# baldhat/yolov10-3D

Hardware: AMD Instinct MI355X
Metric: train_images_per_sec (higher is better)
Workload: dtype bf16

## Files before the change

include/y3d.h:

```cpp
#ifndef Y3D_H
#define Y3D_H
#include <stdint.h>

#ifdef __cplusplus
extern "C" {
#endif

enum { Y3D_F32 = 0, Y3D_BF16 = 1 };
enum { Y3D_OK = 0, Y3D_ERR_INVALID = -1, Y3D_ERR_HIP = -2 };

const char* y3d_last_error(void);
int y3d_abi_version(void);
int y3d_device_info(char* name, int name_len, int* compute_units, int* lds_bytes, int* clock_khz);

int y3d_pack_weight_fwd(int dtype, const float* w_oihw, void* out, int Cout, int Cin_g, int Cin_g_pad, int kh, int kw, void* stream);
int y3d_pack_weight_dgrad(int dtype, const float* w_oihw, void* out, int Cout, int Cin_g, int groups, int kh, int kw, void* stream);
int y3d_mt_pack_weights(int dtype, const int64_t* desc, const int* chunk_tensor, const int* chunk_off, int nchunks, int chunk, void* stream);
int y3d_mt_fp8w_quantize(const int64_t* desc, const int* row_begin, int ntensors, int nrows, void* stream);
int y3d_fp8w_dequantize(const uint8_t* codes, const float* scale, float* w, int rows, int K, void* stream);
int y3d_fp8_quantize_act(const void* x, int64_t xsw, int64_t M, int C, uint8_t* q, uint8_t* s, void* stream);
int y3d_fp8_pack_weight_fwd(const uint8_t* codes, const float* scale, int rows, int Cg, uint8_t* wq, uint8_t* ws, void* stream);
int y3d_conv3x3_fp8_ok(int B, int H, int W, int Cin, int Cout, int groups);
int y3d_conv3x3_fp8_stat_rows(int B, int H, int W);
int y3d_fp8_scale_pitch(int C);
// ... 15 lines not shown
  Y3D_ROUTE_SMALL = 2,
  Y3D_ROUTE_SMALL_S2 = 3,
  Y3D_ROUTE_S2_DGRAD = 4,
  Y3D_ROUTE_TILE8 = 5,
  Y3D_ROUTE_TILE16 = 6,
  Y3D_ROUTE_WIDE3_8 = 7,
  Y3D_ROUTE_WIDE3_16 = 8,
  Y3D_ROUTE_FLAT = 9,
  Y3D_ROUTE_WGRAD_SMALL = 10,
  Y3D_ROUTE_WGRAD_TILE = 11,
  Y3D_ROUTE_WGRAD_STREAM1X1 = 12
};
int y3d_conv2d_route(int dtype, int op, int epi, int B, int H, int W, int Cin, int Cout, int groups, int kh, int kw, int stride, int pad);
int y3d_conv2d_fwd(int dtype, const void* x, int64_t xsb, int64_t xsh, int64_t xsw, int B, int H, int W, int Cin,
                   const void* w_packed, const float* bias, void* y, int64_t ysw, int Ho, int Wo, int Cout, int groups,
                   int kh, int kw, int stride, int pad, float* stat_partials, void* stream);
int y3d_conv2d_fwd_affine(int dtype, const void* x, int64_t xsb, int64_t xsh, int64_t xsw, int B, int H, int W, int Cin,
                          const void* w_packed, const float* scale, const float* shift, int act, void* y, int64_t ysw, int Ho, int Wo,
                          int Cout, int groups, int kh, int kw, int stride, int pad, void* stream);
int y3d_conv2d_fwd_affine_res_ok(int dtype, int B, int H, int W, int Cin, int Cout, int groups, int kh, int kw, int stride, int pad);
int y3d_conv2d_fwd_affine_res(int dtype, const void* x, int64_t xsb, int64_t xsh, int64_t xsw, int B, int H, int W, int Cin,
                              const void* w_packed, const float* scale, const float* shift, int act, const void* res, int64_t rsw, void* y,
                              int64_t ysw, int Ho, int Wo, int Cout, int groups, int kh, int kw, int stride, int pad, void* stream);
int y3d_conv2d_bwd_data(int dtype, const void* dy, int64_t dsb, int64_t dsh, int64_t dsw, int B, int Ho, int Wo, int Cout,
                        const void* w_packed_dgrad, void* dx, int64_t xsw, int H, int W, int Cin, int groups, int kh, int kw,
                        int stride, int pad, void* stream);
int y3d_conv2d_wgrad_splits(int dtype, int B, int Ho, int Wo, int Cout, int Cin_g, int groups, int kh, int kw);
int y3d_conv2d_wgrad_plan(int dtype, int B, int H, int W, int Cin, int Cout, int groups, int kh, int kw, int stride, int pad);
int y3d_set_tile_kernels(int enable);
int y3d_set_stream1x1(int enable);
int y3d_get_stream1x1(void);
int y3d_get_tile_kernels(void);
int y3d_set_bn_wide_slabs(int enable);
int y3d_conv2d_bwd_weight(int dtype, const void* x, int64_t xsb, int64_t xsh, int64_t xsw, int B, int H, int W, int Cin,
                          int Cin_real, const void* dy, int64_t dsw, int Ho, int Wo, int Cout, int groups, int kh, int kw,
                          int stride, int pad, float* slab, int nsplit, float* grad_oihw, int accumulate, void* stream);
int y3d_wgrad_fold(const float* slab, int nsplit, int Cout, int taps, int Cin_g, int Cin_g_real, float* grad_oihw, int accumulate,
                   void* stream);

int y3d_dw_blocks(int64_t M);
int y3d_dw_wgrad_blocks(int64_t M);
int y3d_dw_pack_weight(const float* w_oihw, float* out_taps_c, int C, int kh, int kw, void* stream);
int y3d_dwconv2d_fwd(int dtype, const void* x, int64_t xsb, int64_t xsh, int64_t xsw, int B, int H, int W, int C,
                     const float* w_packed, void* y, int64_t ysw, int Ho, int Wo, int kh, int kw, int stride, int pad,
                     float* stat_partials, void* stream);
int y3d_dwconv2d_fwd_affine(int dtype, const void* x, int64_t xsb, int64_t xsh, int64_t xsw, int B, int H, int W, int C,
                            const float* w_packed, const float* scale, const float* shift, int act, int res_mode, const void* res, int64_t rsw,
                            void* z, int64_t zsw, int Ho, int Wo, int kh, int kw, int stride, int pad, void* stream);
int y3d_dwconv2d_bwd_data(int dtype, const void* dy, int64_t dsb, int64_t dsh, int64_t dsw, int B, int Ho, int Wo, int C,
                          const float* w_packed, void* dx, int64_t xsw, int H, int W, int kh, int kw, int stride, int pad,
                          void* stream);
int y3d_dwconv2d_bwd_weight(int dtype, const void* x, int64_t xsb, int64_t xsh, int64_t xsw, int B, int H, int W, int C,
                            const void* dy, int64_t dsw, int Ho, int Wo, int kh, int kw, int stride, int pad, float* slab,
                            float* grad_oihw, int accumulate, void* stream);
int y3d_dw_wgrad_fold(const float* slab, int nblk, int C, int taps, float* grad_oihw, int accumulate, void* stream);

int y3d_bn_finalize(const float* partials, int nblk, int C, int64_t count, const float* gamma, const float* beta, float eps,
                    float momentum, float* running_mean, float* running_var, float* mean, float* invstd, float* scale,
                    float* shift, void* stream);
int y3d_bn_eval_scale(int C, const float* gamma, const float* beta, const float* running_mean, const float* running_var,
                      float eps, float* scale, float* shift, void* stream);
int y3d_bn_act_fwd(int dtype, const void* y, int64_t ysw, const float* scale, const float* shift, int act, int res_mode,
                   const void* res, int64_t rsw, void* z, int64_t zsw, int64_t P, int C, void* stream);
int y3d_bn_act_fwd_q(const void* y, int64_t ysw, const float* scale, const float* shift, int act, void* z, int64_t zsw, uint8_t* q, uint8_t* s,
                     int64_t P, int C, void* stream);
int y3d_bn_bwd_blocks(int64_t P, int C);
// ... 220 lines not shown
```

yolov10-3d_amd/_lib.py:

```python
from __future__ import annotations

import ctypes
import os
import re

_HERE = os.path.dirname(os.path.abspath(__file__))
LIB_PATH = os.path.join(_HERE, "liby3d_hip.so")
HEADER = os.path.join(os.path.dirname(_HERE), "include", "y3d.h")

F32, BF16 = 0, 1

_CT = {"int": ctypes.c_int, "int64_t": ctypes.c_int64, "float": ctypes.c_float, "double": ctypes.c_double}


class Y3DError(RuntimeError):
    pass


def parse_header(path: str = HEADER):
    src = open(path).read()
    src = re.sub(r"/\*.*?\*/", " ", src, flags=re.S)
    protos = {}
    for m in re.finditer(r"(const\s+char\s*\*|int)\s+(y3d_\w+)\s*\(([^;{]*?)\)\s*;", src, flags=re.S):
        ret, name, args = m.group(1), m.group(2), m.group(3).strip()
        argtypes = []
        if args and args != "void":
            for a in args.split(","):
                a = a.strip()
                if "*" in a:
                    argtypes.append(ctypes.c_void_p)
                else:
                    toks = a.split()
                    t = toks[1] if toks[0] == "const" else toks[0]
                    argtypes.append(_CT[t])
        protos[name] = (ctypes.c_char_p if "char" in ret else ctypes.c_int, argtypes)
    return protos


_PLAIN_INT = {"abi_version", "conv_kpad", "conv_stat_blocks", "conv2d_stat_rows", "conv2d_route", "conv2d_wgrad_splits", "conv2d_wgrad_plan", "set_tile_kernels", "set_stream1x1", "set_bn_wide_slabs", "get_stream1x1", "get_tile_kernels", "dw_blocks", "dw_wgrad_blocks", "bn_bwd_blocks", "proj_blocks", "proj_group_blocks", "proj_group_bn_bwd_blocks", "proj_group_bwd_weight_bn_mfma_blocks", "tal3d_scratch_floats", "tal2d_scratch_floats", "v10_postprocess_scratch_floats", "conv2d_fwd_affine_res_ok", "stem_conv_train_rows", "conv3x3_fp8_ok", "conv3x3_fp8_dgrad_ok", "conv3x3_fp8_stat_rows", "fp8_scale_pitch", "kitti_eval_max_boxes", "det_metrics_max_gts", "det_metrics_max_dets"}


class _Lib:
    def __init__(self):
        if not os.path.exists(LIB_PATH):
            raise Y3DError(
                f"{LIB_PATH} not found: build it with `python yolov10-3d_amd/csrc/build.py` "
                "(or __graft_entry__.build()). There is no CPU / PyTorch fallback for the HIP path.")
        self._dll = ctypes.CDLL(LIB_PATH)
        self.protos = parse_header()
        for name, (ret, argtypes) in self.protos.items():
            fn = getattr(self._dll, name)
            fn.restype = ret
            fn.argtypes = argtypes

    def last_error(self) -> str:
        return (self._dll.y3d_last_error() or b"").decode()

    def __getattr__(self, name):
        if name.startswith("_"):
            raise AttributeError(name)
        fn = getattr(self._dll, "y3d_" + name)
        ret = self.protos["y3d_" + name][0]
        if ret is not ctypes.c_int or name in _PLAIN_INT:
            setattr(self, name, fn)
            return fn

        def call(*a):
            rc = fn(*a)
            if rc != 0:
                raise Y3DError(f"y3d_{name} failed ({rc}): {self.last_error()}")
            return rc

# ... 13 lines not shown
```

yolov10-3d_amd/csrc/conv3x3_wgrad_tile.hip:

```cpp
#include "common.h"
#include <cstdlib>

namespace {

__device__ uint4 y3d_wg_zero_page[4];

struct WG3P {
  const void* x;
  const void* dy;
  float* slab;
  long xsb, xsh, xsw, dsw;
  int B, H, W;
  int Cg, Cn, G;
  int ntx, nty;
  int ntiles, tiles_per_split, nslab;
};

typedef __attribute__((ext_vector_type(8))) short s16x8_t;

template <int OFF>
__device__ __forceinline__ s16x4_t ds_tr16(unsigned a) {
  s16x4_t v;
#ifdef Y3D_WGP_NOLDS
  asm volatile("" : "=v"(v) : "v"(a));
  return v;
#endif
  asm volatile("ds_read_b64_tr_b16 %0, %1 offset:%2" : "=v"(v) : "v"(a), "n"(OFF));
  return v;
}
template <int N>
__device__ __forceinline__ void lds_wait(s16x4_t& a, s16x4_t& b, s16x4_t& c, s16x4_t& d) {
  asm volatile("s_waitcnt lgkmcnt(%4)" : "+v"(a), "+v"(b), "+v"(c), "+v"(d) : "n"(N));
}

template <int N>
__device__ __forceinline__ void lds_wait8(s16x4_t& a, s16x4_t& b, s16x4_t& c, s16x4_t& d, s16x4_t& e, s16x4_t& f, s16x4_t& g, s16x4_t& h) {
  asm volatile("s_waitcnt lgkmcnt(%8)" : "+v"(a), "+v"(b), "+v"(c), "+v"(d), "+v"(e), "+v"(f), "+v"(g), "+v"(h) : "n"(N));
}

template <int TH>
__global__ __launch_bounds__(512) void conv3x3_wgrad_tile_kernel(WG3P p) {
  typedef bf16_t T;
  constexpr int NT = 512;
  constexpr int NPX = TH * 16;
  constexpr int HWD = 18;
  constexpr int NPIXH = (TH + 2) * HWD;
  constexpr int DR = NPX * 16 / NT;
  constexpr int HCH = NPIXH * 8;
  constexpr int HR = (HCH + NT - 1) / NT;
  constexpr int DBYTES = NPX * 256, HBYTES = HR * NT * 16, SBYTES = DBYTES + HBYTES;
  extern __shared__ __attribute__((aligned(16))) char smem[];

  const int tid = threadIdx.x, lane = tid & 63, wave = tid >> 6;
  const int wi = wave >> 1, wj = wave & 1;
  const int g = blockIdx.z, split = blockIdx.y;
  const int slab_i = blockIdx.x % p.nslab, cot = blockIdx.x / p.nslab;
  const int c0 = cot * 128, ci0 = slab_i * 64;
  const T* __restrict__ X = (const T*)p.x;
  const T* __restrict__ D = (const T*)p.dy;
  const T* zero = (const T*)y3d_wg_zero_page;

  int d_row[DR], d_px[DR], d_c[DR];
#pragma unroll
  for (int rd = 0; rd < DR; ++rd) {
    int chunk = rd * NT + tid;
    int pp = chunk >> 4, s = chunk & 15;
    d_row[rd] = pp >> 4;
    d_px[rd] = pp & 15;
    d_c[rd] = (s ^ ((pp & 7) << 1)) * 8;
  }
  int h_y[HR], h_x[HR], h_c[HR];
#pragma unroll
  for (int rd = 0; rd < HR; ++rd) {
    int chunk = rd * NT + tid;
    int P = chunk >> 3, s = chunk & 7;
    h_y[rd] = chunk < HCH ? P / HWD : -100000;
    h_x[rd] = P - (P / HWD) * HWD;
    h_c[rd] = (s ^ (((h_x[rd] >> 1) & 3) << 1)) * 8;
  }
  auto issue = [&](int tile, int buf) {
    int tx = tile % p.ntx;
    int t2 = tile / p.ntx;
    int ty = t2 % p.nty;
    int b = t2 / p.nty;
    const int x0 = tx * 16, y0 = ty * TH;
    char* db = smem + buf * SBYTES;
    char* hb = db + DBYTES;
#pragma unroll
    for (int rd = 0; rd < DR; ++rd) {
// ... 105 lines not shown
          for (int mt = 0; mt < 2; ++mt)
#pragma unroll
            for (int nt = 0; nt < 2; ++nt)
#ifndef Y3D_WGP_NOMFMA
              acc[r * 3 + q][mt][nt] = __builtin_amdgcn_mfma_f32_16x16x32_bf16(fa[mt], fb[nt], acc[r * 3 + q][mt][nt], 0, 0, 0);
#else
              asm volatile("" ::"v"(fa[mt]), "v"(fb[nt]));
#endif
        }
      }
    }
    asm volatile("s_waitcnt vmcnt(0)" ::: "memory");
    __syncthreads();
  }

  const int Ktot = 9 * p.Cg;
  float* slab = p.slab + ((long)split * p.G * p.Cn + (long)g * p.Cn) * Ktot;
#pragma unroll
  for (int tap = 0; tap < 9; ++tap)
#pragma unroll
    for (int mt = 0; mt < 2; ++mt)
#pragma unroll
      for (int nt = 0; nt < 2; ++nt) {
        int ci = ci0 + wj * 32 + nt * 16 + (lane & 15);
#pragma unroll
        for (int rg = 0; rg < 4; ++rg) {
          int co = c0 + wi * 32 + mt * 16 + (lane >> 4) * 4 + rg;
          if (co < p.Cn && ci < p.Cg) slab[(long)co * Ktot + tap * p.Cg + ci] = acc[tap][mt][nt][rg];
        }
      }
}

template <int TH>
int launch_wg(const WG3P& p, int nsplit, hipStream_t st) {
  constexpr int NPX = TH * 16;
  constexpr int HCH = (TH + 2) * 18 * 8;
  constexpr int HR = (HCH + 511) / 512;
  size_t sm = 2 * ((size_t)NPX * 256 + (size_t)HR * 512 * 16);
  static bool attr_set = false;
  if (!attr_set) {
    (void)hipFuncSetAttribute((const void*)conv3x3_wgrad_tile_kernel<TH>, hipFuncAttributeMaxDynamicSharedMemorySize, (int)sm);
    attr_set = true;
  }
  dim3 grid(p.nslab * cdiv(p.Cn, 128), nsplit, p.G);
  hipLaunchKernelGGL((conv3x3_wgrad_tile_kernel<TH>), grid, dim3(512), sm, st, p);
  Y3D_LAUNCH_CHECK();
  return Y3D_OK;
}

}

int y3d_wgrad_tile_height(int dtype, int H, int W, int Cg, int Cn, int kh, int kw, int stride, int pad) {
  if (dtype != Y3D_BF16 || kh != 3 || kw != 3 || stride != 1 || pad != 1) return 0;
  if (Cg % 16 != 0 || Cg < 64 || Cn % 8 != 0 || W < 8) return 0;
  if (H % 8 == 0) return 8;
  if (H % 4 == 0) return 4;
  return 0;
}

int y3d_wgrad_tile_splits(int th, int B, int H, int W, int Cg, int Cn, int G) {
  long ntiles = (long)B * (H / th) * cdiv(W, 16);
  long blocks = (long)cdiv(Cg, 64) * cdiv(Cn, 128) * G;
  const int target8 = 256;
  const long tgt = th == 8 ? target8 : 2 * target8;
  long want = tgt / blocks;
  if (want > ntiles) want = ntiles;
  long slab_bytes = (long)G * Cn * 9 * Cg * 4;
  long cap = (64L << 20) / slab_bytes;
  if (cap < 16) cap = 16;
  if (cap > 256) cap = 256;
  if (want > cap) want = cap;
  if (want < 1) want = 1;
  return (int)want;
}

int y3d_conv3x3_wgrad_tile_launch(int th, const void* x, long xsb, long xsh, long xsw, const void* dy, long dsw, int B, int H, int W, int Cg,
                                  int Cn, int G, float* slab, int nsplit, void* stream) {
// ... 13 lines not shown
```

yolov10-3d_amd/csrc/conv_gemm.hip:

```cpp
#include "common.h"
#include "conv_frag.h"
#include <cstdlib>

namespace {

struct ConvP {
  const void* x;
  const void* w;
  const float* bias;
  const float* scale;
  const float* shift;
  int act;
  void* y;
  float* part;
  long xsb, xsh, xsw;
  long ysw;
  int B, Hg, Wg;
  int Hq, Wq;
  int Cg, Cn, G;
  int kh, kw, stride, pad;
  int Ktot, Kpad;
  int M;
  int ntx, nty;
};
// ... 244 lines not shown
    for (int a = 0; a < TC; ++a)
#pragma unroll
      for (int j = 0; j < 4; ++j) {
        float s = wave_xor_sum16(ssum[a][j]);
        float q = wave_xor_sum16(ssq[a][j]);
        if (lp == 0) {
          int cl = wc * (BC / WC) + a * 16 + lc + j;
          red[(wp * BC + cl) * 2 + 0] = s;
          red[(wp * BC + cl) * 2 + 1] = q;
        }
      }
    __syncthreads();
    if (tid < BC && c0 + tid < p.Cn) {
      float s = 0.f, q = 0.f;
#pragma unroll
      for (int w = 0; w < WP; ++w) { s += red[(w * BC + tid) * 2]; q += red[(w * BC + tid) * 2 + 1]; }
      float* dst = p.part + ((long)tile_x * (p.G * p.Cn) + g * p.Cn + c0 + tid) * 2;
      dst[0] = s;
      dst[1] = q;
    }
  }
}

struct WgradP {
  const void* x;
  const void* dy;
  float* slab;
  long xsb, xsh, xsw;
  long dsw;
  int B, H, W, Ho, Wo;
  int Cg, Cn, G;
  int kh, kw, stride, pad;
  int Ktot, M, nsplit, chunk_px;
};

template <typename T, int W> struct TFrag;
template <int W> struct TFrag<bf16_t, W> {
  typedef bf16x8_t type;
  static constexpr int KSUB_PX = 32;
  static constexpr int PITCH = W * 2 + 32;
  __device__ static __forceinline__ type load(const char* tile, int i0, int k0, int lane) {
    int grp = lane >> 4, li = lane & 15;
    int q = li >> 2, pp = li & 3;
    const char* a0 = tile + (k0 + 4 * grp + q) * PITCH + (i0 + 4 * pp) * 2;
    s16x4_t lo = __builtin_amdgcn_ds_read_tr16_b64_v4i16((s16x4_t __attribute__((address_space(3)))*)(a0));
    s16x4_t hi = __builtin_amdgcn_ds_read_tr16_b64_v4i16((s16x4_t __attribute__((address_space(3)))*)(a0 + 16 * PITCH));
    typedef __attribute__((ext_vector_type(8))) short s16x8_t;
    s16x8_t v = __builtin_shufflevector(lo, hi, 0, 1, 2, 3, 4, 5, 6, 7);
    return __builtin_bit_cast(bf16x8_t, v);
  }
  __device__ static __forceinline__ f32x4_t mma(type a, type b, f32x4_t c) {
    return __builtin_amdgcn_mfma_f32_16x16x32_bf16(a, b, c, 0, 0, 0);
  }
};
template <int W> struct TFrag<float, W> {
  typedef float type;
  static constexpr int KSUB_PX = 4;
  static constexpr int PITCH = W * 4 + 64;
  __device__ static __forceinline__ type load(const char* tile, int i0, int k0, int lane) {
    return *(const float*)(tile + (k0 + (lane >> 4)) * PITCH + (i0 + (lane & 15)) * 4);
  }
  __device__ static __forceinline__ f32x4_t mma(type a, type b, f32x4_t c) {
    return __builtin_amdgcn_mfma_f32_16x16x4f32(a, b, c, 0, 0, 0);
  }
};

template <typename T, int WD, int WX>
__global__ __launch_bounds__(256) void conv_wgrad_kernel(WgradP p) {
  constexpr int CE = TT<T>::CE;
  constexpr int BPK = TT<T>::BKE;
  constexpr int PD = TFrag<T, WD>::PITCH, PX = TFrag<T, WX>::PITCH;
  constexpr int CPD = WD * sizeof(T) / 16, CPX = WX * sizeof(T) / 16;
  constexpr int ND = BPK * CPD / 256 > 0 ? BPK * CPD / 256 : 1;
  constexpr int NX = BPK * CPX / 256 > 0 ? BPK * CPX / 256 : 1;
  constexpr int TA = WD / 32, TB = WX / 32;
  extern __shared__ __attribute__((aligned(16))) char smem[];
  char* sD = smem;
  char* sX = smem + 2 * BPK * PD;

  const int tid = threadIdx.x, lane = tid & 63, wave = tid >> 6;
  const int wi = wave >> 1, wj = wave & 1;
  const int g = blockIdx.z % p.G;
  const int split = blockIdx.z / p.G;
  const int j0 = blockIdx.x * WX;
  const int i0 = blockIdx.y * WD;
  const T* __restrict__ X = (const T*)p.x;
  const T* __restrict__ D = (const T*)p.dy;

  const int mbeg = split * p.chunk_px;
  const int mend = min(p.M, mbeg + p.chunk_px);
  const int nsteps = (mend - mbeg + BPK - 1) / BPK;

  const int ccd = tid % CPD, rd0 = tid / CPD;
  const int ccx = tid % CPX, rx0 = tid / CPX;
  constexpr int RSD = 256 / CPD, RSX = 256 / CPX;
  const bool tdv = BPK * CPD >= 256 || tid < BPK * CPD, txv = BPK * CPX >= 256 || tid < BPK * CPX;
  const int kx = j0 + ccx * CE;
  const bool kx_ok = txv && kx < p.Ktot;
  int tap = 0, ci = 0, tr = 0, tq = 0;
  if (kx_ok) { tap = kx / p.Cg; ci = kx - tap * p.Cg; tr = tap / p.kw; tq = tap - tr * p.kw; }
  const int cd = i0 + ccd * CE;
  const bool cd_ok = tdv && cd < p.Cn;
  const int HW = p.Ho * p.Wo;

  uint4 rd[ND], rx[NX];
  int rb_[NX], rh_[NX], rw_[NX];
#pragma unroll
  for (int i = 0; i < NX; ++i) {
    int m = mbeg + rx0 + RSX * i;
    int b = m / HW;
    int rem = m - b * HW;
    rb_[i] = b;
    rh_[i] = rem / p.Wo;
    rw_[i] = rem - rh_[i] * p.Wo;
  }
  const T* dcol = D + (long)g * p.Cn + cd;
  const T* xcol = X + (long)g * p.Cg + ci + (long)(tr - p.pad) * p.xsh + (long)(tq - p.pad) * p.xsw;
  auto gload = [&](int st) {
// ... 456 lines not shown
  } else {
    size_t sm = 2 * (128 + 32) * 128;
    hipLaunchKernelGGL((conv_gemm_kernel<T, 128, 32, 4, 1, MODE>), dim3(p.ntx * p.nty, ny, p.G), block, sm, st, p);
  }
  Y3D_LAUNCH_CHECK();
  return Y3D_OK;
}

template <typename T, bool DGRAD>
int launch_conv(ConvP p, hipStream_t st) {
  if (DGRAD && p.kh == 3 && p.kw == 3 && p.stride == 2 && p.pad == 1 && p.Cg % TT<T>::CE == 0) return launch_conv_mode<T, 2>(p, st);
  return launch_conv_mode<T, DGRAD ? 1 : 0>(p, st);
}

}

int y3d_conv3x3_tile_route(int dtype, int B, int H, int W, int Cg, int Cn, int G, int kh, int kw, int stride, int pad);
int y3d_conv3x3_flat_tiles(int B, int H, int W);
int y3d_conv3x3_tile_launch(int dtype, int route, const void* x, long xsb, long xsh, long xsw, int B, int H, int W, int Cg, int Cn, int G,
                            const void* w, int Ktot, void* y, long ysw, float* part, int flip, const float* scale, const float* shift, int act,
                            void* stream);

int y3d_wgrad_tile_height(int dtype, int H, int W, int Cg, int Cn, int kh, int kw, int stride, int pad);
int y3d_wgrad_tile_splits(int th, int B, int H, int W, int Cg, int Cn, int G);
int y3d_conv3x3_wgrad_tile_launch(int th, const void* x, long xsb, long xsh, long xsw, const void* dy, long dsw, int B, int H, int W, int Cg,
                                  int Cn, int G, float* slab, int nsplit, void* stream);

int y3d_conv1x1_stream_ok(int dtype, long M, int K, int N, long xsw, int G = 1);
int y3d_conv1x1_stream_launch(const void* x, long xsw, const void* w, int Kpad, const float* bias, const float* scale, const float* shift, int act,
                              void* y, long ysw, float* part, long M, int K, int N, int G, void* stream);
int y3d_wgrad1x1_stream_ok(int dtype, long M, int Cg, int Cn, long xsw, long dsw);
int y3d_wgrad1x1_stream_launch(const void* x, long xsw, const void* dy, long dsw, long M, int Cg, int Cn, float* slab, int nsplit, int chunk_px,
                               void* stream);
int y3d_conv3x3s2_dgrad_ok(int dtype, int B, int Ho, int Wo, int H, int W, int Cout, int Cin, long dsw, long xsw);
int y3d_conv3x3s2_dgrad_launch(const void* dy, long dsw, int B, int Ho, int Wo, int Cout, const void* w_packed_dgrad, int Kpad, void* dx, long xsw,
                               int H, int W, int Cin, void* stream);
int y3d_conv3x3_small_ok(int dtype, int B, int H, int W, int Cin, int Cout, int rows);
int y3d_conv3x3_small_launch(const void* x, long xsb, long xsh, long xsw, int B, int H, int W, int Cin, int Cout, const void* w, int Ktot, void* y,
                             long ysw, float* part, int rows, int flip, const float* scale, const float* shift, int act, const void* res, long rsw,
                             void* stream);
int y3d_conv3x3_small_rows(int B, int H, int W, int Cin, int Cout);
int y3d_conv3x3_small_s2_ok(int dtype, int B, int H, int W, int Cin, int Cout);
int y3d_conv3x3_small_s2_rows(int B, int H, int W, int Cin, int Cout);
int y3d_conv3x3_small_s2_launch(const void* x, long xsb, long xsh, long xsw, int B, int H, int W, int Cin, int Cout, const void* w, int Ktot, void* y,
                                long ysw, float* part, int rows, const float* scale, const float* shift, int act, void* stream);
int y3d_conv1x1_stream_rows(long M, int K, int N, int G = 1);
int y3d_wgrad3x3_small_ok(int dtype, int B, int H, int W, int Cin, int Cout);
int y3d_wgrad3x3_small_splits(int B, int H, int W);
int y3d_wgrad3x3_small_launch(const void* x, long xsb, long xsh, long xsw, const void* dy, long dsw, int B, int H, int W, int Cin, int Cout,
                              float* slab, int nsplit, void* stream);
static inline bool dense_pixels(int B, int H, int W, long sb, long sh, long sw) {
  return (H == 1 || sh == (long)W * sw) && (B == 1 || sb == (long)H * W * sw);
}

static int g_tile_kernels = 1;
extern "C" int y3d_conv2d_wgrad_splits(int dtype, int B, int Ho, int Wo, int Cout, int Cin_g, int groups, int kh, int kw);

static int conv_route(int dtype, int op, int epi, int B, int H, int W, int Ho, int Wo, int Cin, int Cout, int groups, int kh, int kw, int stride,
                      int pad, bool dense, long asw, long bsw, bool cin_full) {
  const int ce = dtype == Y3D_BF16 ? 8 : 4;
  const bool k1 = kh == 1 && kw == 1 && stride == 1 && pad == 0, k3s1 = kh == 3 && kw == 3 && stride == 1 && pad == 1,
             k3s2 = kh == 3 && kw == 3 && stride == 2 && pad == 1;
  if (op == Y3D_OP_FWD) {
    Y3D_CHECK(dtype == Y3D_BF16 || dtype == Y3D_F32, "conv2d_fwd: bad dtype %d", dtype);
    Y3D_CHECK(B > 0 && H > 0 && W > 0 && Cin > 0 && Cout > 0 && groups > 0, "conv2d_fwd: empty shape");
    Y3D_CHECK(Cin % groups == 0 && Cout % groups == 0, "conv2d_fwd: channels not divisible by groups");
// ... 257 lines not shown
  if (route < 0) return route;
  Y3D_CHECK(nsplit >= 1, "conv2d_bwd_weight: nsplit");
  Y3D_CHECK(Cin_real <= Cin && (Cin_real == Cin || groups == 1), "conv2d_bwd_weight: Cin_real");
  if (check_align("conv2d_bwd_weight x", x, xsb, xsh, xsw, ce)) return Y3D_ERR_INVALID;
  Y3D_CHECK(((uintptr_t)dy & 15) == 0 && dsw % ce == 0, "conv2d_bwd_weight: dy alignment");
  WgradP p;
  p.x = x; p.dy = dy; p.slab = slab;
  p.xsb = xsb; p.xsh = xsh; p.xsw = xsw; p.dsw = dsw;
  p.B = B; p.H = H; p.W = W; p.Ho = Ho; p.Wo = Wo;
  p.Cg = Cin / groups; p.Cn = Cout / groups; p.G = groups;
  p.kh = kh; p.kw = kw; p.stride = stride; p.pad = pad;
  p.Ktot = kh * kw * p.Cg; p.M = B * Ho * Wo; p.nsplit = nsplit;
  p.chunk_px = cdiv(cdiv(p.M, nsplit), bpk) * bpk;
  hipStream_t st = (hipStream_t)stream;
  if (route == Y3D_ROUTE_WGRAD_SMALL) {
    int rc = y3d_wgrad3x3_small_launch(x, xsb, xsh, xsw, dy, dsw, B, H, W, Cin, Cout, slab, nsplit, stream);
    if (rc) return rc;
    return launch_wgrad_reduce(slab, grad_oihw, nsplit, Cout, 9, Cin, Cin, accumulate, st);
  }
  if (route == Y3D_ROUTE_WGRAD_TILE) {
    const int th = y3d_wgrad_tile_height(dtype, H, W, p.Cg, p.Cn, kh, kw, stride, pad);
    Y3D_CHECK(nsplit == y3d_wgrad_tile_splits(th, B, H, W, p.Cg, p.Cn, groups), "conv2d_bwd_weight: nsplit must come from y3d_conv2d_wgrad_plan");
    int rc = y3d_conv3x3_wgrad_tile_launch(th, x, xsb, xsh, xsw, dy, dsw, B, H, W, p.Cg, p.Cn, groups, slab, nsplit, stream);
    if (rc) return rc;
    return launch_wgrad_reduce(slab, grad_oihw, nsplit, Cout, kh * kw, p.Cg, p.Cg, accumulate, st);
  }
  if (route == Y3D_ROUTE_WGRAD_STREAM1X1) {
    int rc = y3d_wgrad1x1_stream_launch(x, xsw, dy, dsw, p.M, Cin, Cout, slab, nsplit, p.chunk_px, stream);
    if (rc) return rc;
    return launch_wgrad_reduce(slab, grad_oihw, nsplit, Cout, 1, Cin, Cin, accumulate, st);
  }
  const int wd = wgrad_tile_w(p.Cn), wx = wgrad_tile_w(p.Ktot);
  dim3 grid(cdiv(p.Ktot, wx), cdiv(p.Cn, wd), groups * nsplit);
#define Y3D_WGRAD(T, WD, WX)                                                                                         \
  hipLaunchKernelGGL((conv_wgrad_kernel<T, WD, WX>), grid, dim3(256),                                                  \
                     2 * TT<T>::BKE * (size_t)(TFrag<T, WD>::PITCH + TFrag<T, WX>::PITCH), st, p)
#define Y3D_WGRAD_T(T)                                                                                               \
  do {                                                                                                               \
    if (wd == 128) { if (wx == 128) Y3D_WGRAD(T, 128, 128); else if (wx == 64) Y3D_WGRAD(T, 128, 64); else Y3D_WGRAD(T, 128, 32); } \
    else if (wd == 64) { if (wx == 128) Y3D_WGRAD(T, 64, 128); else if (wx == 64) Y3D_WGRAD(T, 64, 64); else Y3D_WGRAD(T, 64, 32); } \
    else { if (wx == 128) Y3D_WGRAD(T, 32, 128); else if (wx == 64) Y3D_WGRAD(T, 32, 64); else Y3D_WGRAD(T, 32, 32); }    \
  } while (0)
  if (dtype == Y3D_BF16) Y3D_WGRAD_T(bf16_t); else Y3D_WGRAD_T(float);
#undef Y3D_WGRAD_T
#undef Y3D_WGRAD
  Y3D_LAUNCH_CHECK();
  int cg_real = groups == 1 ? Cin_real : p.Cg;
  return launch_wgrad_reduce(slab, grad_oihw, nsplit, Cout, kh * kw, p.Cg, cg_real, accumulate, st);
}

int y3d_wgrad_fold(const float* slab, int nsplit, int Cout, int taps, int Cin_g, int Cin_g_real, float* grad_oihw, int accumulate, void* stream) {
  Y3D_CHECK(slab && grad_oihw && nsplit >= 1 && Cout >= 1 && Cin_g_real >= 1 && Cin_g_real <= Cin_g, "wgrad_fold: bad argument");
  return launch_wgrad_reduce(slab, grad_oihw, nsplit, Cout, taps, Cin_g, Cin_g_real, accumulate, (hipStream_t)stream);
}

int y3d_mt_pack_weights(int dtype, const int64_t* desc, const int* chunk_tensor, const int* chunk_off, int nchunks, int chunk, void* stream) {
  Y3D_CHECK(dtype == Y3D_BF16 || dtype == Y3D_F32, "mt_pack_weights: bad dtype");
  Y3D_CHECK(nchunks >= 1 && chunk >= 256, "mt_pack_weights: empty chunk table");
  hipStream_t st = (hipStream_t)stream;
  if (dtype == Y3D_BF16) hipLaunchKernelGGL(mt_pack_w_kernel<bf16_t>, dim3(nchunks), dim3(256), 0, st, (const long*)desc, chunk_tensor, chunk_off, chunk);
  else hipLaunchKernelGGL(mt_pack_w_kernel<float>, dim3(nchunks), dim3(256), 0, st, (const long*)desc, chunk_tensor, chunk_off, chunk);
  Y3D_LAUNCH_CHECK();
  return Y3D_OK;
}

}
```

yolov10-3d_amd/csrc/wgrad1x1_stream.hip:

```cpp
#include "common.h"

namespace {

struct Wg1P {
  const bf16_t* x;
  const bf16_t* dy;
  float* slab;
  int xsw, dsw;
  int M, Cg, Cn, chunk_px;
  unsigned xbytes, dbytes;
};

template <int N> __device__ __forceinline__ void wg1_wvm() { asm volatile("s_waitcnt vmcnt(%0)" ::"n"(N) : "memory"); }

__device__ __forceinline__ s16x4_t wg1_tr(unsigned a) {
  s16x4_t v;
  asm volatile("ds_read_b64_tr_b16 %0, %1" : "=v"(v) : "v"(a));
  return v;
}
template <int NF>
__device__ __forceinline__ void wg1_wait(s16x4_t (&f)[NF][2]) {
  if constexpr (NF == 2) asm volatile("s_waitcnt lgkmcnt(0)" : "+v"(f[0][0]), "+v"(f[0][1]), "+v"(f[1][0]), "+v"(f[1][1]));
  else if constexpr (NF == 3) asm volatile("s_waitcnt lgkmcnt(0)" : "+v"(f[0][0]), "+v"(f[0][1]), "+v"(f[1][0]), "+v"(f[1][1]), "+v"(f[2][0]), "+v"(f[2][1]));
  else if constexpr (NF == 4) asm volatile("s_waitcnt lgkmcnt(0)" : "+v"(f[0][0]), "+v"(f[0][1]), "+v"(f[1][0]), "+v"(f[1][1]), "+v"(f[2][0]), "+v"(f[2][1]), "+v"(f[3][0]), "+v"(f[3][1]));
  else {
    static_assert(NF == 6, "2, 3, 4 or 6 fragments");
    asm volatile("s_waitcnt lgkmcnt(0)" : "+v"(f[0][0]), "+v"(f[0][1]), "+v"(f[1][0]), "+v"(f[1][1]), "+v"(f[2][0]), "+v"(f[2][1]), "+v"(f[3][0]), "+v"(f[3][1]),
                 "+v"(f[4][0]), "+v"(f[4][1]), "+v"(f[5][0]), "+v"(f[5][1]));
  }
}

template <int WD, int WX, int WDW>
__global__ __launch_bounds__(512) void wgrad1x1_stream_kernel(Wg1P p) {
  constexpr int NS = 4, BPK = 64;
  constexpr int WXW = 8 / WDW;
  constexpr int TA = WD / WDW / 16, TB = WX / WXW / 16;
  static_assert(TA >= 1 && TB >= 1, "wave tile");
  constexpr int CD = WD / 8 + 2, CX = WX / 8 + 2;
  constexpr int PD = CD * 16, PX = CX * 16;
  constexpr int ID = CD, IX = CX;
  constexpr int NI = (ID + IX + 7) / 8;
  constexpr int STAGE = BPK * (PD + PX);
  extern __shared__ __attribute__((aligned(16))) char smem[];
  char* dump = smem + NS * STAGE;
  const int tid = threadIdx.x, lane = tid & 63, wave = __builtin_amdgcn_readfirstlane(tid >> 6);
  const int wi = wave / WXW, wj = wave % WXW;
  const int split = blockIdx.z;
  const int j0 = blockIdx.x * WX, i0 = blockIdx.y * WD;
  const int mbeg = split * p.chunk_px;
  const int mend = min(p.M, mbeg + p.chunk_px);
  const int nsteps = mend > mbeg ? (mend - mbeg + BPK - 1) / BPK : 0;
  const __amdgpu_buffer_rsrc_t rd = __builtin_amdgcn_make_buffer_rsrc((void*)p.dy, 0, (int)p.dbytes, 0x00020000);
  const __amdgpu_buffer_rsrc_t rx = __builtin_amdgcn_make_buffer_rsrc((void*)p.x, 0, (int)p.xbytes, 0x00020000);
  constexpr unsigned OOB = 0xfffffff0u;

  int is_ = 0, i_slot = 0;
  auto issue = [&]() {
    const bool live = is_ < nsteps;
    const int m0 = mbeg + is_ * BPK;
#pragma unroll
    for (int n = 0; n < NI; ++n) {
      const int ii = wave + 8 * n;
      if (ii < ID) {
        const int q = ii * 64 + lane, row = q / CD, col = q - row * CD;
        const int m = m0 + row, c = i0 + col * 8;
        const bool ok = live & (m < mend) & (col < WD / 8) & (c < p.Cn);
        __builtin_amdgcn_raw_ptr_buffer_load_lds(rd, (__attribute__((address_space(3))) void*)(smem + i_slot * STAGE + ii * 1024), 16,
                                                 ok ? (unsigned)(m * p.dsw + c) * 2u : OOB, 0, 0, 0);
      } else if (ii < ID + IX) {
        const int q = (ii - ID) * 64 + lane, row = q / CX, col = q - row * CX;
        const int m = m0 + row, c = j0 + col * 8;
        const bool ok = live & (m < mend) & (col < WX / 8) & (c < p.Cg);
        __builtin_amdgcn_raw_ptr_buffer_load_lds(rx, (__attribute__((address_space(3))) void*)(smem + i_slot * STAGE + BPK * PD + (ii - ID) * 1024), 16,
                                                 ok ? (unsigned)(m * p.xsw + c) * 2u : OOB, 0, 0, 0);
      } else {
        __builtin_amdgcn_raw_ptr_buffer_load_lds(rx, (__attribute__((address_space(3))) void*)dump, 16, OOB, 0, 0, 0);
      }
    }
    ++is_;
    if (++i_slot == NS) i_slot = 0;
  };
// ... 43 lines not shown
    if (++c_slot == NS) c_slot = 0;
  }
  wg1_wvm<0>();
  float* slab = p.slab + (long)split * p.Cn * p.Cg;
#pragma unroll
  for (int a = 0; a < TA; ++a)
#pragma unroll
    for (int b = 0; b < TB; ++b) {
      const int k = j0 + wj * (WX / WXW) + b * 16 + li;
#pragma unroll
      for (int r = 0; r < 4; ++r) {
        const int co = i0 + wi * (WD / WDW) + a * 16 + grp * 4 + r;
        if (co < p.Cn && k < p.Cg) slab[(long)co * p.Cg + k] = acc[a][b][r];
      }
    }
}

template <int WD, int WX, int WDW>
void wg1_launch(const Wg1P& p, dim3 grid, hipStream_t st) {
  constexpr int CD = WD / 8 + 2, CX = WX / 8 + 2;
  const size_t lds = (size_t)4 * 64 * (CD + CX) * 16 + 1024;
  static bool attr = false;
  if (!attr) {
    (void)hipFuncSetAttribute((const void*)wgrad1x1_stream_kernel<WD, WX, WDW>, hipFuncAttributeMaxDynamicSharedMemorySize, 160 * 1024);
    attr = true;
  }
  hipLaunchKernelGGL((wgrad1x1_stream_kernel<WD, WX, WDW>), grid, dim3(512), lds, st, p);
}

}

extern "C" int y3d_get_stream1x1(void);

int y3d_wgrad1x1_stream_ok(int dtype, long M, int Cg, int Cn, long xsw, long dsw) {
  if (!y3d_get_stream1x1() || dtype != Y3D_BF16 || Cg <= 32 || Cn <= 32 || Cg % 8 || Cn % 8) return 0;
  if ((M * xsw + Cg) * 2 >= (1L << 32) - 64 || (M * dsw + Cn) * 2 >= (1L << 32) - 64) return 0;
  return 1;
}

int y3d_wgrad1x1_stream_launch(const void* x, long xsw, const void* dy, long dsw, long M, int Cg, int Cn, float* slab, int nsplit, int chunk_px,
                               void* stream) {
  Wg1P p;
  p.x = (const bf16_t*)x; p.dy = (const bf16_t*)dy; p.slab = slab; p.xsw = (int)xsw; p.dsw = (int)dsw;
  p.M = (int)M; p.Cg = Cg; p.Cn = Cn; p.chunk_px = chunk_px;
  p.xbytes = (unsigned)(((M - 1) * xsw + Cg) * 2);
  p.dbytes = (unsigned)(((M - 1) * dsw + Cn) * 2);
  const int wd = Cn <= 64 ? 64 : 128, wx = Cg <= 64 ? 64 : 128;
  dim3 grid(cdiv(Cg, wx), cdiv(Cn, wd), nsplit);
  hipStream_t st = (hipStream_t)stream;
  if (wd == 128 && wx == 128) wg1_launch<128, 128, 2>(p, grid, st);
  else if (wd == 64 && wx == 128) wg1_launch<64, 128, 2>(p, grid, st);
  else if (wd == 128 && wx == 64) wg1_launch<128, 64, 4>(p, grid, st);
  else wg1_launch<64, 64, 2>(p, grid, st);
  Y3D_LAUNCH_CHECK();
  return Y3D_OK;
}
```

Measured before the change: 1449.

## Remap wgrad block order so each XCD processes all output tiles of a split

Adds an XCD-aware block remapping to three weight-gradient kernels (3x3 tile, generic GEMM wgrad, 1x1 stream). Blocks are linearised so that consecutive groups of 8 map to different splits, which round-robin dispatch places on separate XCDs, while the same XCD sweeps all output tiles of one split. Tiles of a split then share the same input/dy pixel chunk in that XCD's L2. A heuristic gates the remap on load balance. Padding blocks exit early, and some launches may become less balanced.

Result: no change. 1450 (median of 2 runs) (+0.1%).

```diff
diff --git a/include/y3d.h b/include/y3d.h
--- a/include/y3d.h
+++ b/include/y3d.h
@@ -71,6 +71,7 @@
 int y3d_get_stream1x1(void);
 int y3d_get_tile_kernels(void);
 int y3d_set_bn_wide_slabs(int enable);
+int y3d_set_wgrad_xcd_order(int enable);
 int y3d_conv2d_bwd_weight(int dtype, const void* x, int64_t xsb, int64_t xsh, int64_t xsw, int B, int H, int W, int Cin,
                           int Cin_real, const void* dy, int64_t dsw, int Ho, int Wo, int Cout, int groups, int kh, int kw,
                           int stride, int pad, float* slab, int nsplit, float* grad_oihw, int accumulate, void* stream);
diff --git a/yolov10-3d_amd/_lib.py b/yolov10-3d_amd/_lib.py
--- a/yolov10-3d_amd/_lib.py
+++ b/yolov10-3d_amd/_lib.py
@@ -37,7 +37,7 @@
     return protos
 
 
-_PLAIN_INT = {"abi_version", "conv_kpad", "conv_stat_blocks", "conv2d_stat_rows", "conv2d_route", "conv2d_wgrad_splits", "conv2d_wgrad_plan", "set_tile_kernels", "set_stream1x1", "set_bn_wide_slabs", "get_stream1x1", "get_tile_kernels", "dw_blocks", "dw_wgrad_blocks", "bn_bwd_blocks", "proj_blocks", "proj_group_blocks", "proj_group_bn_bwd_blocks", "proj_group_bwd_weight_bn_mfma_blocks", "tal3d_scratch_floats", "tal2d_scratch_floats", "v10_postprocess_scratch_floats", "conv2d_fwd_affine_res_ok", "stem_conv_train_rows", "conv3x3_fp8_ok", "conv3x3_fp8_dgrad_ok", "conv3x3_fp8_stat_rows", "fp8_scale_pitch", "kitti_eval_max_boxes", "det_metrics_max_gts", "det_metrics_max_dets"}
+_PLAIN_INT = {"abi_version", "conv_kpad", "conv_stat_blocks", "conv2d_stat_rows", "conv2d_route", "conv2d_wgrad_splits", "conv2d_wgrad_plan", "set_tile_kernels", "set_stream1x1", "set_bn_wide_slabs", "set_wgrad_xcd_order","get_stream1x1", "get_tile_kernels", "dw_blocks", "dw_wgrad_blocks", "bn_bwd_blocks", "proj_blocks", "proj_group_blocks", "proj_group_bn_bwd_blocks", "proj_group_bwd_weight_bn_mfma_blocks", "tal3d_scratch_floats", "tal2d_scratch_floats", "v10_postprocess_scratch_floats", "conv2d_fwd_affine_res_ok", "stem_conv_train_rows", "conv3x3_fp8_ok", "conv3x3_fp8_dgrad_ok", "conv3x3_fp8_stat_rows", "fp8_scale_pitch", "kitti_eval_max_boxes", "det_metrics_max_gts", "det_metrics_max_dets"}
 
 
 class _Lib:
diff --git a/yolov10-3d_amd/csrc/conv3x3_wgrad_tile.hip b/yolov10-3d_amd/csrc/conv3x3_wgrad_tile.hip
--- a/yolov10-3d_amd/csrc/conv3x3_wgrad_tile.hip
+++ b/yolov10-3d_amd/csrc/conv3x3_wgrad_tile.hip
@@ -1,5 +1,7 @@
 #include "common.h"
 #include <cstdlib>
+
+int y3d_wgrad_xcd_order_for(int T, int Z, int kept);
 
 namespace {
 
@@ -14,6 +16,7 @@
   int Cg, Cn, G;
   int ntx, nty;
   int ntiles, tiles_per_split, nslab;
+  int T, nsplit;
 };
 
 typedef __attribute__((ext_vector_type(8))) short s16x8_t;
@@ -40,6 +43,14 @@
 
 template <int TH>
 __global__ __launch_bounds__(512) void conv3x3_wgrad_tile_kernel(WG3P p) {
+  int g = blockIdx.z, split = blockIdx.y, cb = blockIdx.x;
+  if (p.T) {
+    const int r = blockIdx.x >> 3, u = (r / p.T) * 8 + (blockIdx.x & 7);
+    if (u >= p.nsplit * p.G) return;
+    cb = r % p.T;
+    g = u / p.nsplit;
+    split = u - g * p.nsplit;
+  }
   typedef bf16_t T;
   constexpr int NT = 512;
   constexpr int NPX = TH * 16;
@@ -53,8 +64,7 @@
 
   const int tid = threadIdx.x, lane = tid & 63, wave = tid >> 6;
   const int wi = wave >> 1, wj = wave & 1;
-  const int g = blockIdx.z, split = blockIdx.y;
-  const int slab_i = blockIdx.x % p.nslab, cot = blockIdx.x / p.nslab;
+  const int slab_i = cb % p.nslab, cot = cb / p.nslab;
   const int c0 = cot * 128, ci0 = slab_i * 64;
   const T* __restrict__ X = (const T*)p.x;
   const T* __restrict__ D = (const T*)p.dy;
@@ -226,7 +236,7 @@
 }
 
 template <int TH>
-int launch_wg(const WG3P& p, int nsplit, hipStream_t st) {
+int launch_wg(WG3P p, int nsplit, hipStream_t st) {
   constexpr int NPX = TH * 16;
   constexpr int HCH = (TH + 2) * 18 * 8;
   constexpr int HR = (HCH + 511) / 512;
@@ -237,6 +247,11 @@
     attr_set = true;
   }
   dim3 grid(p.nslab * cdiv(p.Cn, 128), nsplit, p.G);
+  p.T = 0; p.nsplit = nsplit;
+  if (y3d_wgrad_xcd_order_for((int)grid.x, nsplit * p.G, grid.x > 2)) {
+    p.T = (int)grid.x;
+    grid = dim3(8 * p.T * cdiv(nsplit * p.G, 8), 1, 1);
+  }
   hipLaunchKernelGGL((conv3x3_wgrad_tile_kernel<TH>), grid, dim3(512), sm, st, p);
   Y3D_LAUNCH_CHECK();
   return Y3D_OK;
diff --git a/yolov10-3d_amd/csrc/conv_gemm.hip b/yolov10-3d_amd/csrc/conv_gemm.hip
--- a/yolov10-3d_amd/csrc/conv_gemm.hip
+++ b/yolov10-3d_amd/csrc/conv_gemm.hip
@@ -300,6 +300,7 @@
   int Cg, Cn, G;
   int kh, kw, stride, pad;
   int Ktot, M, nsplit, chunk_px;
+  int T, gx;
 };
 
 template <typename T, int W> struct TFrag;
@@ -335,6 +336,14 @@
 
 template <typename T, int WD, int WX>
 __global__ __launch_bounds__(256) void conv_wgrad_kernel(WgradP p) {
+  int bz = blockIdx.z, bx = blockIdx.x, by = blockIdx.y;
+  if (p.T) {
+    const int r = blockIdx.x >> 3, tile = r % p.T;
+    bz = (r / p.T) * 8 + (blockIdx.x & 7);
+    if (bz >= p.G * p.nsplit) return;
+    by = tile / p.gx;
+    bx = tile - by * p.gx;
+  }
   constexpr int CE = TT<T>::CE;
   constexpr int BPK = TT<T>::BKE;
   constexpr int PD = TFrag<T, WD>::PITCH, PX = TFrag<T, WX>::PITCH;
@@ -348,10 +357,10 @@
 
   const int tid = threadIdx.x, lane = tid & 63, wave = tid >> 6;
   const int wi = wave >> 1, wj = wave & 1;
-  const int g = blockIdx.z % p.G;
-  const int split = blockIdx.z / p.G;
-  const int j0 = blockIdx.x * WX;
-  const int i0 = blockIdx.y * WD;
+  const int g = bz % p.G;
+  const int split = bz / p.G;
+  const int j0 = bx * WX;
+  const int i0 = by * WD;
   const T* __restrict__ X = (const T*)p.x;
   const T* __restrict__ D = (const T*)p.dy;
 
@@ -874,6 +883,7 @@
 int y3d_wgrad1x1_stream_ok(int dtype, long M, int Cg, int Cn, long xsw, long dsw);
 int y3d_wgrad1x1_stream_launch(const void* x, long xsw, const void* dy, long dsw, long M, int Cg, int Cn, float* slab, int nsplit, int chunk_px,
                                void* stream);
+int y3d_wgrad_xcd_order_for(int T, int Z, int kept);
 int y3d_conv3x3s2_dgrad_ok(int dtype, int B, int Ho, int Wo, int H, int W, int Cout, int Cin, long dsw, long xsw);
 int y3d_conv3x3s2_dgrad_launch(const void* dy, long dsw, int B, int Ho, int Wo, int Cout, const void* w_packed_dgrad, int Kpad, void* dx, long xsw,
                                int H, int W, int Cin, void* stream);
@@ -1197,7 +1207,12 @@
   }
   const int wd = wgrad_tile_w(p.Cn), wx = wgrad_tile_w(p.Ktot);
   dim3 grid(cdiv(p.Ktot, wx), cdiv(p.Cn, wd), groups * nsplit);
-#define Y3D_WGRAD(T, WD, WX)                                                                                         \
+  p.T = 0; p.gx = (int)grid.x;
+  if (y3d_wgrad_xcd_order_for((int)(grid.x * grid.y), groups * nsplit, dtype == Y3D_BF16 && wd == 128 && wx == 128)) {
+    p.T = (int)(grid.x * grid.y);
+    grid = dim3(8 * p.T * cdiv(groups * nsplit, 8), 1, 1);
+  }
+#define Y3D_WGRAD(T, WD, WX)                                                                                        \
   hipLaunchKernelGGL((conv_wgrad_kernel<T, WD, WX>), grid, dim3(256),                                                  \
                      2 * TT<T>::BKE * (size_t)(TFrag<T, WD>::PITCH + TFrag<T, WX>::PITCH), st, p)
 #define Y3D_WGRAD_T(T)                                                                                               \
diff --git a/yolov10-3d_amd/csrc/wgrad1x1_stream.hip b/yolov10-3d_amd/csrc/wgrad1x1_stream.hip
--- a/yolov10-3d_amd/csrc/wgrad1x1_stream.hip
+++ b/yolov10-3d_amd/csrc/wgrad1x1_stream.hip
@@ -9,6 +9,7 @@
   int xsw, dsw;
   int M, Cg, Cn, chunk_px;
   unsigned xbytes, dbytes;
+  int T, gx, nsplit;
 };
 
 template <int N> __device__ __forceinline__ void wg1_wvm() { asm volatile("s_waitcnt vmcnt(%0)" ::"n"(N) : "memory"); }
@@ -32,6 +33,14 @@
 
 template <int WD, int WX, int WDW>
 __global__ __launch_bounds__(512) void wgrad1x1_stream_kernel(Wg1P p) {
+  int split = blockIdx.z, bx = blockIdx.x, by = blockIdx.y;
+  if (p.T) {
+    const int r = blockIdx.x >> 3, tile = r % p.T;
+    split = (r / p.T) * 8 + (blockIdx.x & 7);
+    if (split >= p.nsplit) return;
+    by = tile / p.gx;
+    bx = tile - by * p.gx;
+  }
   constexpr int NS = 4, BPK = 64;
   constexpr int WXW = 8 / WDW;
   constexpr int TA = WD / WDW / 16, TB = WX / WXW / 16;
@@ -45,8 +54,7 @@
   char* dump = smem + NS * STAGE;
   const int tid = threadIdx.x, lane = tid & 63, wave = __builtin_amdgcn_readfirstlane(tid >> 6);
   const int wi = wave / WXW, wj = wave % WXW;
-  const int split = blockIdx.z;
-  const int j0 = blockIdx.x * WX, i0 = blockIdx.y * WD;
+  const int j0 = bx * WX, i0 = by * WD;
   const int mbeg = split * p.chunk_px;
   const int mend = min(p.M, mbeg + p.chunk_px);
   const int nsteps = mend > mbeg ? (mend - mbeg + BPK - 1) / BPK : 0;
@@ -156,6 +164,22 @@
 
 extern "C" int y3d_get_stream1x1(void);
 
+static int g_wgrad_xcd_order = 1;
+
+extern "C" int y3d_set_wgrad_xcd_order(int enable) {
+  const int old = g_wgrad_xcd_order;
+  g_wgrad_xcd_order = enable == 2 ? 2 : (enable ? 1 : 0);
+  return old;
+}
+
+int y3d_wgrad_xcd_order_for(int T, int Z, int kept) {
+  if (!g_wgrad_xcd_order) return 0;
+  if (g_wgrad_xcd_order == 2) return 1;
+  if (!kept || T < 2) return 0;
+  const int busiest = T * cdiv(Z, 8), natural = cdiv(T * Z, 8);
+  return busiest <= (natural > 32 ? natural : 32);
+}
+
 int y3d_wgrad1x1_stream_ok(int dtype, long M, int Cg, int Cn, long xsw, long dsw) {
   if (!y3d_get_stream1x1() || dtype != Y3D_BF16 || Cg <= 32 || Cn <= 32 || Cg % 8 || Cn % 8) return 0;
   if ((M * xsw + Cg) * 2 >= (1L << 32) - 64 || (M * dsw + Cn) * 2 >= (1L << 32) - 64) return 0;
@@ -171,6 +195,11 @@
   p.dbytes = (unsigned)(((M - 1) * dsw + Cn) * 2);
   const int wd = Cn <= 64 ? 64 : 128, wx = Cg <= 64 ? 64 : 128;
   dim3 grid(cdiv(Cg, wx), cdiv(Cn, wd), nsplit);
+  p.T = 0; p.gx = (int)grid.x; p.nsplit = nsplit;
+  if (y3d_wgrad_xcd_order_for((int)(grid.x * grid.y), nsplit, 1)) {
+    p.T = (int)(grid.x * grid.y);
+    grid = dim3(8 * p.T * cdiv(nsplit, 8), 1, 1);
+  }
   hipStream_t st = (hipStream_t)stream;
   if (wd == 128 && wx == 128) wg1_launch<128, 128, 2>(p, grid, st);
   else if (wd == 64 && wx == 128) wg1_launch<64, 128, 2>(p, grid, st);
```
